# Tencent/PocketFlow

Hardware: AMD Instinct MI355X
Metric: images/sec ResNet-50 INT8 quant-aware fine-tune (whole job; per GPU = value / n_gpus) (higher is better)
Workload: dtype bf16

## Files before the change

### include/pocketflow_hip.h

```cpp
#ifndef POCKETFLOW_HIP_H_
#define POCKETFLOW_HIP_H_

#include <stdint.h>

#ifdef __cplusplus
extern "C" {
#endif

enum { PF_F32 = 0, PF_BF16 = 1 };
enum { PF_ACT_NONE = 0, PF_ACT_RELU = 1, PF_ACT_RELU6 = 2 };
enum { PF_BUCKET_TENSOR = 0, PF_BUCKET_CHANNEL = 1, PF_BUCKET_SPLIT = 2 };

typedef struct PfSeg {
  int64_t offset;
  int64_t len;
  int32_t RS;
  int32_t layout;
  int32_t I, O;
  int32_t mode;
  int32_t bits;
  int32_t bucket_size;
  int32_t n_bucket;
  int64_t slot_offset;
  int64_t cb_offset;
// ... 130 lines not shown

int pf_conv2d_stats_groups_geom(int imgs, int H, int Wd, int C, int N, int th, int tw, int stride, int pad_h, int pad_w,
                                int Ho, int Wo);
int pf_conv2d_fwd(const void* X, const void* W, void* Y, const void* zero, const void* R, float* partial,
                  const void* bn_x, const float* bn_scale_shift, const float* bn_mean_invstd, int bn_act,
                  int imgs, int H, int Wd, int C, int N, int th, int tw, int stride, int pad_h, int pad_w,
                  int Ho, int Wo, void* stream);
int pf_conv2d_fwd_affine(const void* X, const void* W, void* Y, const void* zero, const float* out_scale_shift, int out_act,
                         int imgs, int H, int Wd, int C, int N, int th, int tw, int stride, int pad_h, int pad_w, int Ho, int Wo,
                         void* stream);

int pf_conv2d_wrw_splits(int M, int N, int C, int taps);
int pf_conv2d_wrw(const void* dY, const void* X, void* dW, int dw_dtype, float* workspace, int imgs, int H, int Wd, int C,
                  int N, int th, int tw, int stride, int pad_h, int pad_w, int Ho, int Wo, void* stream);

typedef struct PfTransposeTile {
  int64_t src_off, dst_off;
  int32_t O, I, src_ld, dst_ld;
  int32_t o0, i0;
  int32_t reserved0, reserved1;
} PfTransposeTile;
int pf_seg_transpose(const void* src_flat, void* dst_flat, int dtype, const void* tiles, int n_tiles, void* stream);

int pf_maxpool_fwd(const void* x, void* y, void* idx, int dtype, int B, int H, int W, int C, int k, int stride,
                   int pad_h, int pad_w, int Ho, int Wo, void* stream);
int pf_maxpool_bwd(const void* dy, const void* idx, void* dx, int dtype, int B, int H, int W, int C, int k, int stride,
                   int pad_h, int pad_w, int Ho, int Wo, void* stream);

int pf_conv_stem_supported(int H, int Wd, int C, int N, int k, int stride, int pad);
int pf_conv_stem_fwd(const void* X, const void* W, void* Y, int imgs, int H, int Wd, void* stream);
// ... 101 lines not shown
```

### pocketflow_amd/csrc/pf_conv.hip

```cpp
#include "pf_conv_common.h"

template <int BN_T, bool PRO, bool BWD, bool MAP>
__global__ __launch_bounds__(PF_THREADS, 2) void k_conv1x1_fwd(const ConvArgs a) {
  constexpr int WM = (BN_T == 128) ? 64 : 32;
  constexpr int JM = WM / 16;
  constexpr int CS_LD = BN_T + 8;
  constexpr int VPR = BN_T / 8;
  constexpr int RPP = PF_THREADS / VPR;
  constexpr int NBV = BN_T * 8 / PF_THREADS;
  constexpr int A_EL = CV_BM * CV_LDK, B_EL = BN_T * CV_LDK;
  constexpr int C_EL = CV_BM * CS_LD;
  constexpr int RED_FL = 4 * RPP * BN_T;
  constexpr int SM_BYTES_AB = (A_EL + B_EL) * 2;
  constexpr int SM_BYTES = SM_BYTES_AB > RED_FL * 4 ? (SM_BYTES_AB > C_EL * 2 ? SM_BYTES_AB : C_EL * 2)
                                                    : RED_FL * 4;
  constexpr int SS_BYTES = PRO ? 2 * CV_MAXK * 4 : 0;
  __shared__ __attribute__((aligned(16))) unsigned char smem[SM_BYTES + SS_BYTES];
  float* ssl = reinterpret_cast<float*>(smem + SM_BYTES);
  __shared__ float bpl[BWD ? 4 * BN_T : 4];
  bf16_t* As = reinterpret_cast<bf16_t*>(smem);
  bf16_t* Bs = As + A_EL;
  bf16_t* Cs = reinterpret_cast<bf16_t*>(smem);
  float* red = reinterpret_cast<float*>(smem);

// ... 545 lines not shown
  if (e < n)
    for (int s = s0 + sg; s < s1; s += 4) acc += partial[(int64_t)s * n + e];
  l[sg][e_l] = acc;
  __syncthreads();
  if (sg == 0 && e < n) store_one<TO>(out + (int64_t)blockIdx.y * out_stride + e, (l[0][e_l] + l[1][e_l]) + (l[2][e_l] + l[3][e_l]));
}

WrwPlan pf_wrw_plan(int M, int N, int C, int taps, bool entry_1x1, int64_t x_rows, int window_imgs);
int pf_wrw2_launch(const void* dY, const void* X, float* slabs, const float* scale_shift, int act, const uint32_t* slot,
                   int bits, int M, int N, int C, int th, int tw, int H, int Wd, int Ho, int Wo, int stride, int pad_h,
                   int pad_w, int S, int64_t x_rows, hipStream_t st);
int pf_wrw_tr_launch(const void* dY, const void* X, float* slabs, const float* scale_shift, int act,
                     const uint32_t* slot, int bits, int M, int N, int C, int th, int tw, int H, int Wd, int Ho, int Wo,
                     int stride, int pad_h, int pad_w, int S, hipStream_t st);

int pf_wrw_reduce(float* workspace, int S, int64_t n, void* dW, int dw_dtype, hipStream_t st) {
  const int gx = (int)((n + 63) / 64);
  int ry = 1;
  while (ry < 32 && gx * ry < 1024 && ry * 8 <= S) ry *= 2;
  float* stage = workspace + (int64_t)S * n;
  if (ry > 1) {
    k_wrw_reduce<float><<<dim3(gx, ry), PF_THREADS, 0, st>>>(workspace, S, n, stage, n);
    if (dw_dtype == PF_F32) k_wrw_reduce<float><<<dim3(gx, 1), PF_THREADS, 0, st>>>(stage, ry, n, (float*)dW, 0);
    else if (dw_dtype == PF_BF16) k_wrw_reduce<bf16_t><<<dim3(gx, 1), PF_THREADS, 0, st>>>(stage, ry, n, (bf16_t*)dW, 0);
    else return (int)hipErrorInvalidValue;
  } else {
    if (dw_dtype == PF_F32) k_wrw_reduce<float><<<dim3(gx, 1), PF_THREADS, 0, st>>>(workspace, S, n, (float*)dW, 0);
    else if (dw_dtype == PF_BF16) k_wrw_reduce<bf16_t><<<dim3(gx, 1), PF_THREADS, 0, st>>>(workspace, S, n, (bf16_t*)dW, 0);
    else return (int)hipErrorInvalidValue;
  }
  PF_LAUNCH_CHECK();
  return 0;
}

int pf_wrw_scatter_splits(int M, int N, int K) {
  const int tiles = ((N + WR_TN - 1) / WR_TN) * ((K + WR_TK - 1) / WR_TK);
  int S = (768 + tiles - 1) / tiles;
  const int maxS = (M + 4 * WR_BM - 1) / (4 * WR_BM);
  if (S > maxS) S = maxS;
  if (S < 1) S = 1;
  int rows = (M + S - 1) / S;
  rows = ((rows + WR_BM - 1) / WR_BM) * WR_BM;
  return (M + rows - 1) / rows;
}

extern "C" int pf_conv1x1_wrw_splits(int M, int N, int K) { return pf_wrw_plan(M, N, K, 1, true, 0, 0).S; }

extern "C" int pf_conv1x1_wrw(const void* dY, const void* X, void* dW, int dw_dtype, float* workspace,
                              const float* scale_shift, int act, const uint32_t* slot, int bits, int M, int N,
                              int K, int Ho, int Wo, int H, int Wd, int stride, void* stream) {
  if (M <= 0 || N <= 0 || K <= 0 || (K % 8) || (N % 8) || ((int64_t)N * K) % 4) return (int)hipErrorInvalidValue;
  if (!pf_aligned16(dY) || !pf_aligned16(X) || !pf_aligned16(workspace) || !pf_aligned16(dW))
    return (int)hipErrorInvalidValue;
  if (slot != nullptr && (bits < 1 || bits > 32 || scale_shift == nullptr)) return (int)hipErrorInvalidValue;
  if (stride < 1) stride = 1;
  hipStream_t st = (hipStream_t)stream;
  if (stride > 1 && (Ho <= 0 || Wo <= 0 || H <= 0 || Wd <= 0)) return (int)hipErrorInvalidValue;
  const int64_t x_rows = (stride > 1) ? (int64_t)(M / (Ho * Wo)) * H * Wd : (int64_t)M;
  const WrwPlan p = pf_wrw_plan(M, N, K, 1, true, x_rows, 0);
  int r = 0;
  if (p.kernel == WRW_SHARED) {
    r = pf_wrw2_launch(dY, X, workspace, scale_shift, act, slot, bits, M, N, K, 1, 1, H, Wd, Ho, Wo, stride, 0, 0, p.S, x_rows, st);
  } else if (p.kernel == WRW_WAVE) {
    r = pf_wrw_tr_launch(dY, X, workspace, scale_shift, act, slot, bits, M, N, K, 1, 1, H, Wd, Ho, Wo, stride, 0, 0, p.S, st);
  } else {
    ConvArgs a = conv_args(X, dY, nullptr, M, N, K);
    conv_args_prologue(a, scale_shift, act, slot, bits);
    conv_args_rowmap(a, Ho, Wo, H, Wd, stride, 0);
    a.partial = workspace;
    a.tiles_n = (N + WR_TN - 1) / WR_TN;
    const int tiles_k = (K + WR_TK - 1) / WR_TK;
    int rows = (M + p.S - 1) / p.S;
    rows = ((rows + WR_BM - 1) / WR_BM) * WR_BM;
    a.rows_per_split = rows;
    dim3 grid(a.tiles_n * tiles_k, p.S);
    if (scale_shift != nullptr) k_conv1x1_wrw<true><<<grid, PF_THREADS, 0, st>>>(a);
    else k_conv1x1_wrw<false><<<grid, PF_THREADS, 0, st>>>(a);
    PF_LAUNCH_CHECK();
  }
  if (r != 0) return r;
  return pf_wrw_reduce(workspace, p.S, (int64_t)N * K, dW, dw_dtype, st);
}
```

### pocketflow_amd/csrc/pf_stem.hip

```cpp
#include "pf_conv_common.h"

#define LDS_PTR(p) ((__attribute__((address_space(3))) void*)(p))
typedef short st_v4s __attribute__((ext_vector_type(4)));
typedef short st_v8s __attribute__((ext_vector_type(8)));
#if defined(__HIP_DEVICE_COMPILE__)
typedef __amdgpu_buffer_rsrc_t st_rsrc_t;
#define ST_MAKE_RSRC(p, bytes) __builtin_amdgcn_make_buffer_rsrc((void*)(p), (short)0, (int)(bytes), 0x00020000)
#define ST_BUFFER_LOAD_LDS16(rs, lds, voff) __builtin_amdgcn_raw_ptr_buffer_load_lds(rs, LDS_PTR(lds), 16, voff, 0, 0, 0)
#else
typedef int st_rsrc_t;
#define ST_MAKE_RSRC(p, bytes) 0
#define ST_BUFFER_LOAD_LDS16(rs, lds, voff) ((void)(rs), (void)(lds), (void)(voff))
#endif

#define ST_THREADS 256
#define ST_OROWS 8
#define ST_IROWS (2 * ST_OROWS + 5)
#define ST_N 64
#define ST_R 7
#define ST_WL_BYTES (ST_N * ST_R * 32 * 2)

struct StemArgs {
  const bf16_t* X;
  const bf16_t* W;
// ... 240 lines not shown
}

int pf_wrw_reduce(float* workspace, int S, int64_t n, void* dW, int dw_dtype, hipStream_t st);

static int stem_wrw_grid(int imgs, int H) {
  const int items = imgs * ((H / 2 + SW_OROWS - 1) / SW_OROWS);
  return items < 768 ? items : 768;
}

extern "C" int pf_conv_stem_wrw_slabs(int imgs, int H, int Wd) {
  if (!pf_conv_stem_supported(H, Wd, 3, ST_N, 7, 2, 3) || imgs <= 0 || Wd > 256) return 0;
  if ((int64_t)imgs * (H / 2) * (Wd / 2) * ST_N * 2 >= (int64_t)1 << 31) return 0;
  return stem_wrw_grid(imgs, H);
}

extern "C" int pf_conv_stem_wrw(const void* dY, const void* X, void* dW, int dw_dtype, float* workspace, int imgs, int H,
                                int Wd, void* stream) {
  const int S = pf_conv_stem_wrw_slabs(imgs, H, Wd);
  if (S <= 0 || workspace == nullptr) return (int)hipErrorInvalidValue;
  if (!pf_aligned16(dY) || (reinterpret_cast<uintptr_t>(X) & 3u)) return (int)hipErrorInvalidValue;
  StemWrwArgs a;
  a.dY = (const bf16_t*)dY; a.X = (const bf16_t*)X; a.slabs = workspace;
  a.imgs = imgs; a.H = H; a.Wd = Wd; a.Ho = H / 2; a.Wo = Wd / 2;
  a.strips = (a.Ho + SW_OROWS - 1) / SW_OROWS;
  a.n_items = imgs * a.strips;
  a.rsb = (Wd + 8) * 8;
  a.dy_bytes = (int)((int64_t)imgs * a.Ho * a.Wo * ST_N * 2);
  const size_t lds = (size_t)SW_IROWS * a.rsb + (size_t)SW_OROWS * a.Wo * ST_N * 2;
  if (int e = pf_require_lds(reinterpret_cast<const void*>(&k_stem7x7_wrw), lds)) return e;
  k_stem7x7_wrw<<<S, ST_THREADS, lds, (hipStream_t)stream>>>(a);
  PF_LAUNCH_CHECK();
  return pf_wrw_reduce(workspace, S, (int64_t)ST_N * 147, dW, dw_dtype, (hipStream_t)stream);
}
```

### pocketflow_amd/csrc/pf_wrw.hip

```cpp
#include "pf_conv_common.h"
#include <stdlib.h>

#define LDS_PTR(p) ((__attribute__((address_space(3))) void*)(p))
typedef short v4s __attribute__((ext_vector_type(4)));
typedef short v8s __attribute__((ext_vector_type(8)));

__device__ __attribute__((aligned(16))) const uint32_t pf_wrw_zero_page[64] = {0};

struct WrwArgs {
  const bf16_t* dY;
  const bf16_t* X;
  float* slabs;
  const float* ss;
  const uint32_t* slot;
  float kq, act_lo, act_hi;
  int M, N, C;
  int th, tw, H, Wd, Ho, Wo, stride, pad_h, pad_w;
  int tiles_n, tiles, rows_per_split;
};

template <int N> __device__ __forceinline__ void wrw_wait_vm() { asm volatile("s_waitcnt vmcnt(%0)" ::"n"(N) : "memory"); }

template <int BN, bool PRO, bool MAP>
__global__ __launch_bounds__(256) void k_wrw_tr(const WrwArgs a) {
// ... 612 lines not shown
  const int s1 = (!entry_1x1 || pf_tuning().wrw_tr != 0) ? wrw_tr_splits(M, N, C, taps) : 0;
  if (s1 > 0) return WrwPlan{WRW_WAVE, s1};
  if (entry_1x1) return WrwPlan{WRW_SCATTER, pf_wrw_scatter_splits(M, N, C)};
  return WrwPlan{WRW_NONE, 0};
}

extern "C" int pf_conv2d_wrw_splits(int M, int N, int C, int taps) {
  const int s = pf_wrw_plan(M, N, C, taps, false, 0, 0).S;
  if (pf_tuning().conv3x3_c64 != 0 && taps == 9 && N == 64 && C == 64 && M % (56 * 56) == 0) {
    const int s3 = pf_wrw_plan(M, N, C, taps, false, 0, M / (56 * 56)).S;
    return s3 > s ? s3 : s;
  }
  return s;
}

extern "C" int pf_conv2d_wrw(const void* dY, const void* X, void* dW, int dw_dtype, float* workspace, int imgs, int H,
                             int Wd, int C, int N, int th, int tw, int stride, int pad_h, int pad_w, int Ho, int Wo,
                             void* stream) {
  if (imgs <= 0 || H <= 0 || Wd <= 0 || Ho <= 0 || Wo <= 0 || th < 1 || tw < 1 || stride < 1) return (int)hipErrorInvalidValue;
  if (!pf_aligned16(dY) || !pf_aligned16(X) || !pf_aligned16(dW) || !pf_aligned16(workspace)) return (int)hipErrorInvalidValue;
  const int M = imgs * Ho * Wo;
  hipStream_t st = (hipStream_t)stream;
  const bool window = pf_wrw3x3_c64_geom(H, Wd, C, N, th, tw, stride, pad_h, pad_w, Ho, Wo);
  const WrwPlan p = pf_wrw_plan(M, N, C, th * tw, false, (int64_t)imgs * H * Wd, window ? imgs : 0);
  int r = (int)hipErrorInvalidValue;
  if (p.kernel == WRW_WINDOW) r = pf_wrw3x3_c64_launch(dY, X, workspace, imgs, st);
  if (p.kernel == WRW_SHARED)
    r = pf_wrw2_launch(dY, X, workspace, nullptr, PF_ACT_NONE, nullptr, 8, M, N, C, th, tw, H, Wd, Ho, Wo, stride, pad_h, pad_w, p.S,
                       (int64_t)imgs * H * Wd, st);
  if (p.kernel == WRW_WAVE)
    r = pf_wrw_tr_launch(dY, X, workspace, nullptr, PF_ACT_NONE, nullptr, 8, M, N, C, th, tw, H, Wd, Ho, Wo, stride, pad_h, pad_w, p.S, st);
  if (r != 0) return r;
  return pf_wrw_reduce(workspace, p.S, (int64_t)N * th * tw * C, dW, dw_dtype, st);
}
```

### pocketflow_amd/graph.py

```python
from __future__ import annotations

import contextlib
import math
import os
import weakref
import threading
from dataclasses import dataclass, field
from typing import Callable, Dict, List, Optional, Sequence, Tuple

import numpy as np
import torch
import torch.nn.functional as F

from pocketflow_amd import hip
from pocketflow_amd.hip import check_gather
from pocketflow_amd.plan import WeightDesc
from pocketflow_amd.profiling import region

ALIGN = 64
FUSE_BN_BWD_STATS = os.environ.get('PF_FUSE_BN_BWD_STATS', '1') != '0'
HEAD_FUSE = os.environ.get('PF_HEAD_FUSE', '1') != '0'
HEAD_FUSE_ANY_DEVICE = False
BN_JOIN_ANY_DEVICE = False

# ... 62 lines not shown
      return WeightDesc(self.name, self.offset, s[0] * s[1], s[2], 1, 1)
    raise ValueError('not a matmul kernel: %s' % self.name)


class VarStore:

  def __init__(self, scope: str):
    self.scope = scope
    self.vars: List[Variable] = []
    self.by_name: Dict[str, Variable] = {}
    self.finalized = False
    self.device = None
    self.compute_dtype = torch.float32
    self.weight_decay = 0.0
    self.grad_hook = None

  def add(self, name: str, ref_shape, kind: str, trainable: bool = True, l2: bool = True,
          init=None) -> Variable:
    full = self.scope + '/' + name if self.scope else name
    if full in self.by_name:
      return self.by_name[full]
    if self.finalized:
      raise RuntimeError('variable %s created after the store was finalized' % full)
    v = Variable(full, tuple(int(d) for d in ref_shape), kind, trainable, l2 and trainable, init)
    v.numel = int(np.prod(v.ref_shape))
    v.group = 'W' if kind in ('conv', 'dense', 'depthwise') else ('O' if trainable else 'S')
    v.store = self
    self.vars.append(v)
    self.by_name[full] = v
    return v
# ... 307 lines not shown



WRW_SIDE = os.environ.get('PF_WRW_SIDE', '1') != '0'


class WrwSide(object):

  def __init__(self, device):
    self.device = device
    self.stream = torch.cuda.Stream(device=device)
    self.keep: List = []
    self._scratch: Optional[torch.Tensor] = None
    self.armed = False
    self.forks = 0

  def scratch(self, n_floats: int) -> torch.Tensor:
    if self._scratch is None or self._scratch.numel() < n_floats:
      with torch.cuda.stream(self.stream):
        self._scratch = torch.empty(max(n_floats, 1 << 20), dtype=torch.float32, device=self.device)
    return self._scratch

  def join(self) -> None:
    if self.forks:
      torch.cuda.current_stream(self.device).wait_stream(self.stream)
    self.keep.clear()
    self.forks = 0


class _WrwQueue(object):

  def __init__(self, graph, direct, tensors):
    side = getattr(getattr(graph, 'store', None), 'wrw_side', None)
    self.side = side if (side is not None and side.armed and direct and not torch.cuda.is_current_stream_capturing()) else None
    self.graph, self.tensors, self.ctx = graph, tensors, None

  def __enter__(self):
    if self.side is None:
      return self.graph.scratch
    side = self.side
    side.stream.wait_stream(torch.cuda.current_stream(side.device))
    side.keep.append(self.tensors)
    side.forks += 1
    self.ctx = torch.cuda.stream(side.stream)
    self.ctx.__enter__()
    return side.scratch

  def __exit__(self, *exc):
    if self.ctx is not None:
      self.ctx.__exit__(*exc)
    return False


def _wrw_queue(graph, direct, *tensors):
  return _WrwQueue(graph, direct, tensors)


@contextlib.contextmanager
def wrw_side_armed(store: 'VarStore'):
  if not (WRW_SIDE and store is not None and getattr(store, 'device', None) is not None and torch.device(store.device).type == 'cuda'):
    yield
    return
  side = getattr(store, 'wrw_side', None)
  if side is None:
    side = store.wrw_side = WrwSide(store.device)
  side.armed = True
  try:
    yield
  finally:
    side.armed = False
    side.join()



def _nhwc(x: torch.Tensor) -> torch.Tensor:
  if x.dim() == 4:
    return x.contiguous(memory_format=torch.channels_last)
  return x.contiguous()


def _bn_fast_ok(C: int) -> bool:
  if C % 8:
    return False
  G = C // 8
  if G < 8:
    return 8 % G == 0
# ... 399 lines not shown
  gview = _grad_view(params[0], C) if params is not None else None
  bview = _grad_view(params[1], C) if params is not None else None
  direct = gview is not None and bview is not None
  dgamma = gview if direct else torch.empty(C, dtype=torch.float32, device=x.device)
  dbeta = bview if direct else torch.empty(C, dtype=torch.float32, device=x.device)
  hip.bn_bwd_finalize(partial, nblk, C, dgamma, dbeta)
  dx = torch.empty_like(x)
  zero = graph.zero_row(C)[:C] if frozen else None
  name, traffic, launch, hw, tail = apply_pass
  with region(name, traffic):
    launch(dq, x, dx, rows, C, *hw, scale_shift, mean_invstd, zero if frozen else dgamma, zero if frozen else dbeta, act,
           *tail)
  return (dx, None, None) if direct else (dx, dgamma, dbeta)


def _filter_grad(graph, w, w_var, keep, name, nbytes, launch):
  gw = getattr(w, 'grad', None)
  direct = gw is not None and gw.shape == w.shape and gw.dtype == w.dtype and gw.permute(0, 2, 3, 1).is_contiguous()
  target = (gw.permute(0, 2, 3, 1) if direct
            else torch.empty((w.shape[0], w.shape[2], w.shape[3], w.shape[1]), dtype=w.dtype, device=w.device))
  with _wrw_queue(graph, direct, *keep) as scratch, region(name, nbytes):
    launch(target, scratch)
    if direct:
      graph.store.notify_grad(w_var)
  return None if direct else target.permute(0, 3, 1, 2)


def _bwd_data_weight(graph, w_var, w):
  if USE_SEG_TRANSPOSE and w_var is not None and w_var.store is graph.store and w_var.tensor is w:
    return graph.store.transposed(w_var)
  return w.detach().permute(0, 2, 3, 1).flip(1, 2).permute(3, 1, 2, 0).contiguous()


def _krsc(w, dtype):
  wk = w.detach().permute(0, 2, 3, 1)
  if not wk.is_contiguous() or wk.dtype != dtype:
    wk = wk.contiguous().to(dtype)
  return wk

# ... 61 lines not shown
  @staticmethod
  def backward(ctx, dy):
    x, w2d = ctx.saved_tensors
    lazy, stride, graph, has_res, w_shape = ctx.meta
    dy = _nhwc(dy)
    N, K = w2d.shape
    M, geom, _ = _conv1x1_geom(x.shape, stride)
    ss = lazy.scale_shift if lazy is not None else None
    quant = lazy is not None and lazy.bits is not None
    act = lazy.act if lazy is not None else None
    dx = dw = None
    if ctx.needs_input_grad[1]:
      S = hip.conv1x1_wrw_splits(M, N, K)

      def wrw(dwk, scratch):
        hip.conv1x1_wrw(dy, x, dwk.view(N, K), scratch((S + 32) * N * K), M, N, K, scale_shift=ss, act=act,
                        slot=lazy.slot if quant else None, bits=lazy.bits if quant else 8, geom=geom)
      dw = _filter_grad(graph, ctx.w_leaf, ctx.w_var, (dy, x, w2d, ss, lazy), 'conv1x1_wrw', float((M * K + M * N) * 2), wrw)
    if ctx.needs_input_grad[0]:
      wt = _bwd_data_weight(graph, ctx.w_var, ctx.w_leaf).view(K, N)
      fuse_stats = (FUSE_BN_BWD_STATS and lazy is not None and lazy.n_consumers == 1 and geom is None
                    and lazy.mean_invstd is not None and lazy.act in ('Relu', 'Relu6'))
      join = (JOIN_TWO_CONSUMERS and lazy is not None and lazy.join_ok and lazy.n_consumers == 2
              and lazy.n_grad_consumers == 2)
      second = join and lazy.pending is not None
      res = lazy.pending if (second and geom is None) else None
      join_entry = getattr(hip, 'conv1x1_bwd_data_join', None) if PROJ_JOIN else None
      compact = (join and not second and geom is not None and join_entry is not None and lazy.dense_out is not None
                 and hip.conv1x1_join_plan(x.shape[0] * x.shape[2] * x.shape[3], lazy.dense_out, K) != 0)
      rgeom = lazy.pending_geom if res is not None else None
      join_stats = (res is not None and join_entry is not None and PROJ_JOIN_STATS and FUSE_BN_BWD_STATS
                    and lazy.mean_invstd is not None and lazy.act in ('Relu', 'Relu6')
                    and hip.conv1x1_join_plan(M, N, K, True) != 0)
# ... 89 lines not shown

  @staticmethod
  def backward(ctx, dy):
    x, w = ctx.saved_tensors
    stride, pad, graph, bn_box = ctx.meta
    dy = _nhwc(dy)
    dx = dw = None
    N, C, R, S = w.shape
    B, _, H, W = x.shape
    Ho, Wo = dy.shape[2], dy.shape[3]
    if ctx.needs_input_grad[1]:
      splits = hip.conv2d_wrw_splits(B * Ho * Wo, N, C, R * S) if (OWN_CONV2D_WRW and C >= OWN_CONV2D_WRW_MIN_C) else 0
      nbytes = float((x.numel() + dy.numel()) * 2)
      if splits > 0:
        def wrw(dwk, scratch):
          hip.conv2d_wrw(dy, x, dwk, scratch((splits + 32) * N * R * S * C), B, H, W, C, N, R, S, stride, pad[0], pad[1], Ho, Wo)
        dw = _filter_grad(graph, w, ctx.w_var, (dy, x), 'conv2d_wrw', nbytes, wrw)
      elif OWN_CONV2D_WRW and OWN_CONV_GENERIC and x.is_cuda and dy.dtype == x.dtype and w.dtype == x.dtype:
        gs = hip.convg_wrw_splits(B, C, N, R, S, Ho, Wo)
        dwk = torch.empty((N, R, S, C), dtype=w.dtype, device=x.device)
        with region('conv2d_wrw', nbytes):
          hip.convg_wrw(dy, x, dwk, graph.scratch(gs * N * R * S * C), B, H, W, C, N, R, S, stride, pad[0], pad[1], Ho, Wo)
        dw = dwk.permute(0, 3, 1, 2)
      else:
        with region('conv2d_wrw', nbytes):
          dw = torch.ops.aten.convolution_backward(dy, x, w.detach(), None, [stride, stride], list(pad), [1, 1], False,
                                                   [0, 0], 1, [False, True, False])[1]
    if ctx.needs_input_grad[0]:
      mfma = N % 64 == 0 and C % 8 == 0 and igemm_limits_ok(dy.numel(), w.numel(), R * S)
      by_classes = (OWN_CONV2D_BWD_STRIDED and stride > 1 and H % stride == 0 and W % stride == 0 and R >= stride and S >= stride
                    and dy.dtype == torch.bfloat16)
      if mfma and (stride == 1 or by_classes):
# ... 158 lines not shown
    ctx.meta = (graph, w_var)
    return _run_stem(x, w)

  @staticmethod
  def backward(ctx, dy):
    x, w = ctx.saved_tensors
    graph, w_var = ctx.meta
    dy = _nhwc(dy)
    dx = dw = None
    if ctx.needs_input_grad[1]:
      B, _, H, Wd = x.shape
      S = hip.conv_stem_wrw_slabs(B, H, Wd) if OWN_CONV2D_WRW else 0
      nbytes = float((x.numel() + dy.numel()) * 2)
      if S > 0:
        def wrw(dwk, scratch):
          hip.conv_stem_wrw(dy, x, dwk, scratch((S + 32) * 64 * 147), B, H, Wd)
        dw = _filter_grad(graph, w, w_var, (dy, x), 'conv_stem_wrw', nbytes, wrw)
      else:
        with region('conv_stem_wrw', nbytes):
          dw = torch.ops.aten.convolution_backward(dy, x, w.detach(), None, [2, 2], [3, 3], [1, 1], False, [0, 0], 1,
                                                   [False, True, False])[1]
    if ctx.needs_input_grad[0]:
      dx = torch.ops.aten.convolution_backward(dy, x, w.detach(), None, [2, 2], [3, 3], [1, 1], False, [0, 0], 1,
                                               [True, False, False])[0]
    return dx, dw, None, None


def _run_stem3(x, w, pads, out_hw):
  B, _, H, Wd = x.shape
  N = w.shape[0]
  Ho, Wo = out_hw
  y = torch.empty((B, N, Ho, Wo), dtype=x.dtype, device=x.device, memory_format=torch.channels_last)
# ... 754 lines not shown
```

### pocketflow_amd/hip.py

```python
from __future__ import annotations

import ctypes
import os
from ctypes import c_float, c_int, c_int64, c_void_p

import numpy as np
import torch

_LIB_PATH = os.environ.get('PF_HIP_LIB') or os.path.join(os.path.dirname(os.path.abspath(__file__)), 'csrc', 'libpocketflow_hip.so')

PF_F32, PF_BF16 = 0, 1
PF_ACT_NONE, PF_ACT_RELU, PF_ACT_RELU6 = 0, 1, 2
PF_BUCKET_TENSOR, PF_BUCKET_CHANNEL, PF_BUCKET_SPLIT = 0, 1, 2
PF_CHUNK = 4096

SEG_DTYPE = np.dtype([('offset', '<i8'), ('len', '<i8'), ('RS', '<i4'), ('layout', '<i4'),
                      ('I', '<i4'), ('O', '<i4'), ('mode', '<i4'), ('bits', '<i4'),
                      ('bucket_size', '<i4'), ('n_bucket', '<i4'), ('slot_offset', '<i8'),
                      ('cb_offset', '<i8')])
BLOCK_DTYPE = np.dtype([('seg', '<i4'), ('chunk', '<i4'), ('row0', '<i4'), ('nrows', '<i4')])
assert SEG_DTYPE.itemsize == 64 and BLOCK_DTYPE.itemsize == 16

ACT_CODES = {None: PF_ACT_NONE, 'none': PF_ACT_NONE, 'Relu': PF_ACT_RELU, 'relu': PF_ACT_RELU,
             'Relu6': PF_ACT_RELU6, 'relu6': PF_ACT_RELU6}
# ... 12 lines not shown
    'pf_depthwise_wrw', 'pf_conv2d_stats_groups_geom', 'pf_tuning_reload',
    'pf_adam_flat_dev', 'pf_momentum_flat_dev', 'pf_set_floats',
    'pf_convg_fwd', 'pf_convg_bwd_data', 'pf_convg_small_splits', 'pf_convg_wrw_splits', 'pf_convg_wrw', 'pf_conv2d_bwd_data_strided',
    'pf_prox_groups', 'pf_prox_norms', 'pf_prox_apply', 'pf_im2col', 'pf_col2im',
    'pf_conv_stem3_supported', 'pf_conv_stem3_fwd', 'pf_conv_stem3_wrw_slabs', 'pf_conv_stem3_wrw',
    'pf_conv1x1_fwd_affine', 'pf_conv2d_fwd_affine', 'pf_conv2d_bwd_data_strided_stats_groups',
    'pf_conv2d_bwd_data_strided_bnstats',
    'pf_cpr_gather', 'pf_cpr_gram_ws', 'pf_cpr_gram', 'pf_cpr_ista', 'pf_cpr_lstsq_splits', 'pf_cpr_lstsq_step', 'pf_cpr_lstsq_resid',
    'pf_conv_gather_fwd',
    'pf_conv1x1_join_plan', 'pf_conv1x1_bwd_data_join',
    'pf_bn_act_quant_pool', 'pf_bn_bwd_stats_pooled', 'pf_bn_bwd_apply_pooled', 'pf_ce_distill_head', 'pf_ce_combine',
    'pf_bn_act_quant_codes', 'pf_conv_i8_supported', 'pf_conv_i8_fwd',
    'pf_dw_i8_supported', 'pf_dw_i8_fwd',
    'pf_bn_act_quant_static', 'pf_conv_i8_fwd_q', 'pf_dw_i8_fwd_q',
    'pf_bn_add_act_groups', 'pf_bn_add_act_fwd', 'pf_bn_add_act_bwd_gate', 'pf_bn_add_act_bwd_gate_add',
]


class HipLibraryMissing(RuntimeError):
  pass


def lib_path() -> str:
  return _LIB_PATH


def _load() -> ctypes.CDLL:
  if not os.path.exists(_LIB_PATH):
    raise HipLibraryMissing(
        'pocketflow_amd: %s not found -- build it with `python -c "import __graft_entry__ as g; '
# ... 412 lines not shown
  Ho, Wo, H, Wd, stride = geom if geom is not None else (0, 0, 0, 0, 1)
  if out_scale_shift is not None:
    if R is not None or partial is not None or slot is not None or ymap:
      raise ValueError('the folded output pass takes no residual, statistics, quantiser or row map')
    _check(_lib.pf_conv1x1_fwd_affine(_ptr(X), _ptr(W), _ptr(Y), _ptr(scale_shift), c_int(ACT_CODES[act]), _ptr(out_scale_shift),
                                      c_int(ACT_CODES[out_act]), c_int(M), c_int(N), c_int(K), c_int(Ho), c_int(Wo), c_int(H),
                                      c_int(Wd), c_int(stride), _stream()), 'pf_conv1x1_fwd_affine')
    return
  _check(_lib.pf_conv1x1_fwd(_ptr(X), _ptr(W), _ptr(Y), _ptr(R), _ptr(scale_shift), c_int(ACT_CODES[act]),
                             _ptr(slot), c_int(int(bits)), _ptr(partial), c_int(M), c_int(N), c_int(K), c_int(Ho),
                             c_int(Wo), c_int(H), c_int(Wd), c_int(stride), c_int(1 if ymap else 0), _stream()),
         'pf_conv1x1_fwd')


def conv1x1_wrw(dY, X, dW, workspace, M: int, N: int, K: int, scale_shift=None, act=None, slot=None,
                bits: int = 8, geom=None) -> None:
  _dev(X)
  Ho, Wo, H, Wd, stride = geom if geom is not None else (0, 0, 0, 0, 1)
  _check(_lib.pf_conv1x1_wrw(_ptr(dY), _ptr(X), _ptr(dW), c_int(dtype_code(dW)), _ptr(workspace), _ptr(scale_shift),
                             c_int(ACT_CODES[act]), _ptr(slot), c_int(int(bits)), c_int(M), c_int(N), c_int(K),
                             c_int(Ho), c_int(Wo), c_int(H), c_int(Wd), c_int(stride), _stream()), 'pf_conv1x1_wrw')


def conv1x1_bwd_data_bnstats(dY, Wt, dQ, bn_x, bn_scale_shift, bn_mean_invstd, bn_act, partial, M: int, N: int,
                             K: int) -> None:
  _dev(dY)
  _check(_lib.pf_conv1x1_bwd_data_bnstats(_ptr(dY), _ptr(Wt), _ptr(dQ), _ptr(bn_x), _ptr(bn_scale_shift),
                                          _ptr(bn_mean_invstd), c_int(ACT_CODES[bn_act]), _ptr(partial), c_int(M),
                                          c_int(N), c_int(K), _stream()), 'pf_conv1x1_bwd_data_bnstats')


def conv1x1_join_plan(M: int, N: int, K: int, with_stats: bool = False) -> int:
  return int(_lib.pf_conv1x1_join_plan(c_int(M), c_int(N), c_int(K), c_int(1 if with_stats else 0)))
# ... 38 lines not shown
                                     c_int(ACT_CODES[out_act]), c_int(imgs), c_int(H), c_int(Wd), c_int(C), c_int(N), c_int(th),
                                     c_int(tw), c_int(stride), c_int(pad_h), c_int(pad_w), c_int(Ho), c_int(Wo), _stream()),
           'pf_conv2d_fwd_affine')
    return
  _check(_lib.pf_conv2d_fwd(_ptr(X), _ptr(W), _ptr(Y), _ptr(zero_page(X.device)), _ptr(R), _ptr(partial), _ptr(bn_x),
                            _ptr(bn_scale_shift), _ptr(bn_mean_invstd), c_int(ACT_CODES[bn_act]), c_int(imgs), c_int(H),
                            c_int(Wd), c_int(C), c_int(N), c_int(th), c_int(tw), c_int(stride), c_int(pad_h),
                            c_int(pad_w), c_int(Ho), c_int(Wo), _stream()), 'pf_conv2d_fwd')


def conv2d_wrw_splits(M: int, N: int, C: int, taps: int) -> int:
  return int(_lib.pf_conv2d_wrw_splits(c_int(M), c_int(N), c_int(C), c_int(taps)))


def conv2d_wrw(dY, X, dW, workspace, imgs: int, H: int, Wd: int, C: int, N: int, th: int, tw: int, stride: int,
               pad_h: int, pad_w: int, Ho: int, Wo: int) -> None:
  _dev(X)
  _check(_lib.pf_conv2d_wrw(_ptr(dY), _ptr(X), _ptr(dW), c_int(dtype_code(dW)), _ptr(workspace), c_int(imgs), c_int(H),
                            c_int(Wd), c_int(C), c_int(N), c_int(th), c_int(tw), c_int(stride), c_int(pad_h),
                            c_int(pad_w), c_int(Ho), c_int(Wo), _stream()), 'pf_conv2d_wrw')


def depthwise_supported(C: int, k: int, stride: int) -> bool:
  return bool(_lib.pf_depthwise_supported(c_int(C), c_int(k), c_int(stride)))


def depthwise_groups(B: int, Ho: int, Wo: int, C: int) -> int:
  return int(_lib.pf_depthwise_groups(c_int(B), c_int(Ho), c_int(Wo), c_int(C)))


def depthwise_fwd(X, W, Y, B: int, H: int, Wd: int, C: int, k: int, stride: int, pad_h: int, pad_w: int, Ho: int, Wo: int,
                  partial=None) -> None:
  _dev(X)
  _check(_lib.pf_depthwise_fwd(_ptr(X), _ptr(W), _ptr(Y), c_int(dtype_code(X)), _ptr(partial), c_int(B), c_int(H), c_int(Wd),
                               c_int(C), c_int(k), c_int(stride), c_int(pad_h), c_int(pad_w), c_int(Ho), c_int(Wo),
# ... 258 lines not shown


def conv_stem_supported(H: int, Wd: int, C: int, N: int, k: int, stride: int, pad: int) -> bool:
  return bool(_lib.pf_conv_stem_supported(c_int(H), c_int(Wd), c_int(C), c_int(N), c_int(k), c_int(stride), c_int(pad)))


def conv_stem_fwd(X, W, Y, imgs: int, H: int, Wd: int) -> None:
  _dev(X)
  _check(_lib.pf_conv_stem_fwd(_ptr(X), _ptr(W), _ptr(Y), c_int(imgs), c_int(H), c_int(Wd), _stream()), 'pf_conv_stem_fwd')


def conv_stem_wrw_slabs(imgs: int, H: int, Wd: int) -> int:
  return int(_lib.pf_conv_stem_wrw_slabs(c_int(imgs), c_int(H), c_int(Wd)))


def conv_stem_wrw(dY, X, dW, workspace, imgs: int, H: int, Wd: int) -> None:
  _dev(dY)
  _check(_lib.pf_conv_stem_wrw(_ptr(dY), _ptr(X), _ptr(dW), c_int(dtype_code(dW)), _ptr(workspace), c_int(imgs), c_int(H),
                               c_int(Wd), _stream()), 'pf_conv_stem_wrw')


def conv_stem3_supported(H: int, Wd: int, C: int, N: int, k: int, stride: int, pad_h: int, pad_w: int, Ho: int, Wo: int) -> bool:
  return bool(_lib.pf_conv_stem3_supported(c_int(H), c_int(Wd), c_int(C), c_int(N), c_int(k), c_int(stride), c_int(pad_h), c_int(pad_w),
                                           c_int(Ho), c_int(Wo)))


def conv_stem3_fwd(X, W, Y, imgs: int, H: int, Wd: int, N: int, pad_h: int, pad_w: int, Ho: int, Wo: int) -> None:
  _dev(X)
  _check(_lib.pf_conv_stem3_fwd(_ptr(X), _ptr(W), _ptr(Y), c_int(imgs), c_int(H), c_int(Wd), c_int(N), c_int(pad_h), c_int(pad_w),
                                c_int(Ho), c_int(Wo), _stream()), 'pf_conv_stem3_fwd')


# ... 39 lines not shown
```

Before: 11710.

## Defer weight-gradient slab reductions into a batched multi-segment reduce kernel

Weight-gradient kernels (1x1, generic conv2d, stem) now only write per-split partial slabs into a pooled arena, and the final split reductions are queued and executed together in one batched kernel that walks a segment table. This replaces one or two small reduce launches per conv layer with a few large launches, cutting launch overhead and tail underutilisation. It costs extra arena memory (up to a configurable MB limit) and delays gradient availability until flush, which disables the path when grad hooks are present and may reduce overlap with the side stream.

```diff
diff --git a/include/pocketflow_hip.h b/include/pocketflow_hip.h
--- a/include/pocketflow_hip.h
+++ b/include/pocketflow_hip.h
@@ -168,6 +168,22 @@
 int pf_conv2d_wrw(const void* dY, const void* X, void* dW, int dw_dtype, float* workspace, int imgs, int H, int Wd, int C,
                   int N, int th, int tw, int stride, int pad_h, int pad_w, int Ho, int Wo, void* stream);
 
+typedef struct PfWrwSeg {
+  const float* slabs;
+  void* out;
+  int64_t n;
+  int32_t S;
+  int32_t dtype;
+} PfWrwSeg;
+int pf_conv1x1_wrw_write(const void* dY, const void* X, float* workspace, const float* scale_shift, int act,
+                         const uint32_t* slot, int bits, int M, int N, int K, int Ho, int Wo, int H, int Wd, int stride,
+                         int* S_out, void* stream);
+int pf_conv2d_wrw_write(const void* dY, const void* X, float* workspace, int imgs, int H, int Wd, int C, int N, int th, int tw,
+                        int stride, int pad_h, int pad_w, int Ho, int Wo, int* S_out, void* stream);
+int pf_conv_stem_wrw_write(const void* dY, const void* X, float* workspace, int imgs, int H, int Wd, void* stream);
+int pf_wrw_reduce_slabs(float* workspace, int S, int64_t n, void* dW, int dw_dtype, void* stream);
+int pf_wrw_reduce_batch(const PfWrwSeg* segs, int count, void* stream);
+
 typedef struct PfTransposeTile {
   int64_t src_off, dst_off;
   int32_t O, I, src_ld, dst_ld;
diff --git a/pocketflow_amd/csrc/pf_conv.hip b/pocketflow_amd/csrc/pf_conv.hip
--- a/pocketflow_amd/csrc/pf_conv.hip
+++ b/pocketflow_amd/csrc/pf_conv.hip
@@ -583,10 +583,112 @@
                      const uint32_t* slot, int bits, int M, int N, int C, int th, int tw, int H, int Wd, int Ho, int Wo,
                      int stride, int pad_h, int pad_w, int S, hipStream_t st);
 
-int pf_wrw_reduce(float* workspace, int S, int64_t n, void* dW, int dw_dtype, hipStream_t st) {
+#define WRB_SEGS 64
+struct WrwSegDev { const float* slabs; void* out; int64_t n; int S; int ry_dtype; };
+struct WrwBatchArgs { WrwSegDev seg[WRB_SEGS]; int wg_end[WRB_SEGS]; int count; };
+
+__device__ __forceinline__ float4 add4(float4 a, float4 b) { return make_float4(a.x + b.x, a.y + b.y, a.z + b.z, a.w + b.w); }
+
+__device__ __forceinline__ float4 wrb_range(const float* __restrict__ p, int64_t n, int s0, int s1) {
+  float4 l0 = make_float4(0.f, 0.f, 0.f, 0.f), l1 = l0, l2 = l0, l3 = l0;
+  int s = s0;
+#pragma unroll 2
+  for (; s + 4 <= s1; s += 4) {
+    const float4 v0 = *reinterpret_cast<const float4*>(p + (int64_t)s * n);
+    const float4 v1 = *reinterpret_cast<const float4*>(p + (int64_t)(s + 1) * n);
+    const float4 v2 = *reinterpret_cast<const float4*>(p + (int64_t)(s + 2) * n);
+    const float4 v3 = *reinterpret_cast<const float4*>(p + (int64_t)(s + 3) * n);
+    l0 = add4(l0, v0); l1 = add4(l1, v1); l2 = add4(l2, v2); l3 = add4(l3, v3);
+  }
+  if (s < s1) l0 = add4(l0, *reinterpret_cast<const float4*>(p + (int64_t)s * n));
+  if (s + 1 < s1) l1 = add4(l1, *reinterpret_cast<const float4*>(p + (int64_t)(s + 1) * n));
+  if (s + 2 < s1) l2 = add4(l2, *reinterpret_cast<const float4*>(p + (int64_t)(s + 2) * n));
+  return add4(add4(l0, l1), add4(l2, l3));
+}
+
+__global__ __launch_bounds__(PF_THREADS) void k_wrw_reduce_batch(const WrwBatchArgs a) {
+  __shared__ float4 l[4][64];
+  const int b = blockIdx.x;
+  int lo = 0, hi = a.count - 1;
+  while (lo < hi) {
+    const int mid = (lo + hi) >> 1;
+    if (b < a.wg_end[mid]) hi = mid; else lo = mid + 1;
+  }
+  const WrwSegDev sg = a.seg[lo];
+  const int wg = b - (lo > 0 ? a.wg_end[lo - 1] : 0);
+  const int lane = threadIdx.x & 63, w = threadIdx.x >> 6;
+  const int64_t e = ((int64_t)wg * 64 + lane) * 4;
+  const int ry = sg.ry_dtype & 0xFF;
+  float4 acc = make_float4(0.f, 0.f, 0.f, 0.f);
+  if (e < sg.n) {
+    const float* __restrict__ p = sg.slabs + e;
+    if (ry == 1) {
+      int s = w;
+      for (; s + 12 < sg.S; s += 16) {
+        const float4 v0 = *reinterpret_cast<const float4*>(p + (int64_t)s * sg.n);
+        const float4 v1 = *reinterpret_cast<const float4*>(p + (int64_t)(s + 4) * sg.n);
+        const float4 v2 = *reinterpret_cast<const float4*>(p + (int64_t)(s + 8) * sg.n);
+        const float4 v3 = *reinterpret_cast<const float4*>(p + (int64_t)(s + 12) * sg.n);
+        acc = add4(add4(add4(add4(acc, v0), v1), v2), v3);
+      }
+      for (; s < sg.S; s += 4) acc = add4(acc, *reinterpret_cast<const float4*>(p + (int64_t)s * sg.n));
+    } else {
+      const int per = (sg.S + ry - 1) / ry;
+      for (int y = w; y < ry; y += 4) {
+        const int s0 = y * per, s1 = (s0 + per < sg.S) ? (s0 + per) : sg.S;
+        acc = add4(acc, wrb_range(p, sg.n, s0, s1));
+      }
+    }
+  }
+  l[w][lane] = acc;
+  __syncthreads();
+  if (w == 0 && e < sg.n) {
+    const float4 r = add4(add4(l[0][lane], l[1][lane]), add4(l[2][lane], l[3][lane]));
+    if ((sg.ry_dtype >> 8) == PF_F32) {
+      *reinterpret_cast<float4*>((float*)sg.out + e) = r;
+    } else {
+      uint2 o;
+      o.x = (uint32_t)f32_to_bf16(r.x) | ((uint32_t)f32_to_bf16(r.y) << 16);
+      o.y = (uint32_t)f32_to_bf16(r.z) | ((uint32_t)f32_to_bf16(r.w) << 16);
+      *reinterpret_cast<uint2*>((bf16_t*)sg.out + e) = o;
+    }
+  }
+}
+
+static int wrw_reduce_ranges(int S, int64_t n) {
   const int gx = (int)((n + 63) / 64);
   int ry = 1;
   while (ry < 32 && gx * ry < 1024 && ry * 8 <= S) ry *= 2;
+  return ry;
+}
+
+extern "C" int pf_wrw_reduce_batch(const PfWrwSeg* segs, int count, void* stream) {
+  if (count < 0 || (count > 0 && segs == nullptr)) return (int)hipErrorInvalidValue;
+  for (int i = 0; i < count; ++i) {
+    const PfWrwSeg& s = segs[i];
+    if (s.S < 1 || s.n <= 0 || (s.n % 4) || (s.n + 255) / 256 > 0x3FFFFF || !pf_aligned16(s.slabs) || !pf_aligned16(s.out) ||
+        (s.dtype != PF_F32 && s.dtype != PF_BF16))
+      return (int)hipErrorInvalidValue;
+  }
+  for (int i0 = 0; i0 < count; i0 += WRB_SEGS) {
+    WrwBatchArgs a;
+    a.count = (count - i0 < WRB_SEGS) ? (count - i0) : WRB_SEGS;
+    int wgs = 0;
+    for (int i = 0; i < WRB_SEGS; ++i) {
+      const PfWrwSeg& s = segs[i0 + (i < a.count ? i : 0)];
+      a.seg[i] = WrwSegDev{s.slabs, s.out, s.n, s.S, wrw_reduce_ranges(s.S, s.n) | (s.dtype << 8)};
+      if (i < a.count) wgs += (int)((s.n + 255) / 256);
+      a.wg_end[i] = wgs;
+    }
+    k_wrw_reduce_batch<<<wgs, PF_THREADS, 0, (hipStream_t)stream>>>(a);
+    PF_LAUNCH_CHECK();
+  }
+  return 0;
+}
+
+int pf_wrw_reduce(float* workspace, int S, int64_t n, void* dW, int dw_dtype, hipStream_t st) {
+  const int gx = (int)((n + 63) / 64);
+  const int ry = wrw_reduce_ranges(S, n);
   float* stage = workspace + (int64_t)S * n;
   if (ry > 1) {
     k_wrw_reduce<float><<<dim3(gx, ry), PF_THREADS, 0, st>>>(workspace, S, n, stage, n);
@@ -602,6 +704,11 @@
   return 0;
 }
 
+extern "C" int pf_wrw_reduce_slabs(float* workspace, int S, int64_t n, void* dW, int dw_dtype, void* stream) {
+  if (S < 1 || n <= 0 || (n % 4) || !pf_aligned16(workspace) || !pf_aligned16(dW)) return (int)hipErrorInvalidValue;
+  return pf_wrw_reduce(workspace, S, n, dW, dw_dtype, (hipStream_t)stream);
+}
+
 int pf_wrw_scatter_splits(int M, int N, int K) {
   const int tiles = ((N + WR_TN - 1) / WR_TN) * ((K + WR_TK - 1) / WR_TK);
   int S = (768 + tiles - 1) / tiles;
@@ -615,12 +722,11 @@
 
 extern "C" int pf_conv1x1_wrw_splits(int M, int N, int K) { return pf_wrw_plan(M, N, K, 1, true, 0, 0).S; }
 
-extern "C" int pf_conv1x1_wrw(const void* dY, const void* X, void* dW, int dw_dtype, float* workspace,
-                              const float* scale_shift, int act, const uint32_t* slot, int bits, int M, int N,
-                              int K, int Ho, int Wo, int H, int Wd, int stride, void* stream) {
+extern "C" int pf_conv1x1_wrw_write(const void* dY, const void* X, float* workspace, const float* scale_shift, int act,
+                                    const uint32_t* slot, int bits, int M, int N, int K, int Ho, int Wo, int H, int Wd,
+                                    int stride, int* S_out, void* stream) {
   if (M <= 0 || N <= 0 || K <= 0 || (K % 8) || (N % 8) || ((int64_t)N * K) % 4) return (int)hipErrorInvalidValue;
-  if (!pf_aligned16(dY) || !pf_aligned16(X) || !pf_aligned16(workspace) || !pf_aligned16(dW))
-    return (int)hipErrorInvalidValue;
+  if (!pf_aligned16(dY) || !pf_aligned16(X) || !pf_aligned16(workspace) || S_out == nullptr) return (int)hipErrorInvalidValue;
   if (slot != nullptr && (bits < 1 || bits > 32 || scale_shift == nullptr)) return (int)hipErrorInvalidValue;
   if (stride < 1) stride = 1;
   hipStream_t st = (hipStream_t)stream;
@@ -648,5 +754,15 @@
     PF_LAUNCH_CHECK();
   }
   if (r != 0) return r;
-  return pf_wrw_reduce(workspace, p.S, (int64_t)N * K, dW, dw_dtype, st);
-}
+  *S_out = p.S;
+  return 0;
+}
+
+extern "C" int pf_conv1x1_wrw(const void* dY, const void* X, void* dW, int dw_dtype, float* workspace,
+                              const float* scale_shift, int act, const uint32_t* slot, int bits, int M, int N,
+                              int K, int Ho, int Wo, int H, int Wd, int stride, void* stream) {
+  if (!pf_aligned16(dW)) return (int)hipErrorInvalidValue;
+  int S = 0;
+  if (int r = pf_conv1x1_wrw_write(dY, X, workspace, scale_shift, act, slot, bits, M, N, K, Ho, Wo, H, Wd, stride, &S, stream)) return r;
+  return pf_wrw_reduce(workspace, S, (int64_t)N * K, dW, dw_dtype, (hipStream_t)stream);
+}
diff --git a/pocketflow_amd/csrc/pf_stem.hip b/pocketflow_amd/csrc/pf_stem.hip
--- a/pocketflow_amd/csrc/pf_stem.hip
+++ b/pocketflow_amd/csrc/pf_stem.hip
@@ -278,8 +278,7 @@
   return stem_wrw_grid(imgs, H);
 }
 
-extern "C" int pf_conv_stem_wrw(const void* dY, const void* X, void* dW, int dw_dtype, float* workspace, int imgs, int H,
-                                int Wd, void* stream) {
+extern "C" int pf_conv_stem_wrw_write(const void* dY, const void* X, float* workspace, int imgs, int H, int Wd, void* stream) {
   const int S = pf_conv_stem_wrw_slabs(imgs, H, Wd);
   if (S <= 0 || workspace == nullptr) return (int)hipErrorInvalidValue;
   if (!pf_aligned16(dY) || (reinterpret_cast<uintptr_t>(X) & 3u)) return (int)hipErrorInvalidValue;
@@ -294,5 +293,11 @@
   if (int e = pf_require_lds(reinterpret_cast<const void*>(&k_stem7x7_wrw), lds)) return e;
   k_stem7x7_wrw<<<S, ST_THREADS, lds, (hipStream_t)stream>>>(a);
   PF_LAUNCH_CHECK();
-  return pf_wrw_reduce(workspace, S, (int64_t)ST_N * 147, dW, dw_dtype, (hipStream_t)stream);
-}
+  return 0;
+}
+
+extern "C" int pf_conv_stem_wrw(const void* dY, const void* X, void* dW, int dw_dtype, float* workspace, int imgs, int H,
+                                int Wd, void* stream) {
+  if (int r = pf_conv_stem_wrw_write(dY, X, workspace, imgs, H, Wd, stream)) return r;
+  return pf_wrw_reduce(workspace, pf_conv_stem_wrw_slabs(imgs, H, Wd), (int64_t)ST_N * 147, dW, dw_dtype, (hipStream_t)stream);
+}
diff --git a/pocketflow_amd/csrc/pf_wrw.hip b/pocketflow_amd/csrc/pf_wrw.hip
--- a/pocketflow_amd/csrc/pf_wrw.hip
+++ b/pocketflow_amd/csrc/pf_wrw.hip
@@ -650,11 +650,10 @@
   return s;
 }
 
-extern "C" int pf_conv2d_wrw(const void* dY, const void* X, void* dW, int dw_dtype, float* workspace, int imgs, int H,
-                             int Wd, int C, int N, int th, int tw, int stride, int pad_h, int pad_w, int Ho, int Wo,
-                             void* stream) {
+extern "C" int pf_conv2d_wrw_write(const void* dY, const void* X, float* workspace, int imgs, int H, int Wd, int C, int N, int th,
+                                   int tw, int stride, int pad_h, int pad_w, int Ho, int Wo, int* S_out, void* stream) {
   if (imgs <= 0 || H <= 0 || Wd <= 0 || Ho <= 0 || Wo <= 0 || th < 1 || tw < 1 || stride < 1) return (int)hipErrorInvalidValue;
-  if (!pf_aligned16(dY) || !pf_aligned16(X) || !pf_aligned16(dW) || !pf_aligned16(workspace)) return (int)hipErrorInvalidValue;
+  if (!pf_aligned16(dY) || !pf_aligned16(X) || !pf_aligned16(workspace) || S_out == nullptr) return (int)hipErrorInvalidValue;
   const int M = imgs * Ho * Wo;
   hipStream_t st = (hipStream_t)stream;
   const bool window = pf_wrw3x3_c64_geom(H, Wd, C, N, th, tw, stride, pad_h, pad_w, Ho, Wo);
@@ -667,5 +666,15 @@
   if (p.kernel == WRW_WAVE)
     r = pf_wrw_tr_launch(dY, X, workspace, nullptr, PF_ACT_NONE, nullptr, 8, M, N, C, th, tw, H, Wd, Ho, Wo, stride, pad_h, pad_w, p.S, st);
   if (r != 0) return r;
-  return pf_wrw_reduce(workspace, p.S, (int64_t)N * th * tw * C, dW, dw_dtype, st);
-}
+  *S_out = p.S;
+  return 0;
+}
+
+extern "C" int pf_conv2d_wrw(const void* dY, const void* X, void* dW, int dw_dtype, float* workspace, int imgs, int H,
+                             int Wd, int C, int N, int th, int tw, int stride, int pad_h, int pad_w, int Ho, int Wo,
+                             void* stream) {
+  if (!pf_aligned16(dW)) return (int)hipErrorInvalidValue;
+  int S = 0;
+  if (int r = pf_conv2d_wrw_write(dY, X, workspace, imgs, H, Wd, C, N, th, tw, stride, pad_h, pad_w, Ho, Wo, &S, stream)) return r;
+  return pf_wrw_reduce(workspace, S, (int64_t)N * th * tw * C, dW, dw_dtype, (hipStream_t)stream);
+}
diff --git a/pocketflow_amd/graph.py b/pocketflow_amd/graph.py
--- a/pocketflow_amd/graph.py
+++ b/pocketflow_amd/graph.py
@@ -100,6 +100,7 @@
     self.compute_dtype = torch.float32
     self.weight_decay = 0.0
     self.grad_hook = None
+    self.wrw_deferred = 0
 
   def add(self, name: str, ref_shape, kind: str, trainable: bool = True, l2: bool = True,
           init=None) -> Variable:
@@ -437,6 +438,7 @@
     self._scratch: Optional[torch.Tensor] = None
     self.armed = False
     self.forks = 0
+    self.arena: Optional['WrwArena'] = None
 
   def scratch(self, n_floats: int) -> torch.Tensor:
     if self._scratch is None or self._scratch.numel() < n_floats:
@@ -445,16 +447,95 @@
     return self._scratch
 
   def join(self) -> None:
+    if self.arena is not None and self.arena.pending and self.arena.side is self:
+      with torch.cuda.stream(self.stream):
+        self.arena.flush()
     if self.forks:
       torch.cuda.current_stream(self.device).wait_stream(self.stream)
     self.keep.clear()
     self.forks = 0
 
 
+WRW_BATCH = os.environ.get('PF_WRW_BATCH', '1') != '0'
+WRW_BATCH_MB = float(os.environ.get('PF_WRW_BATCH_MB', '128'))
+
+
+class _ArenaFull(Exception):
+  pass
+
+
+class WrwArena(object):
+
+  CHUNK = 64 << 20
+
+  def __init__(self, store):
+    self.store = store
+    self.chunks: List[torch.Tensor] = []
+    self.cur = self.off = 0
+    self.pending: List[tuple] = []
+    self.pending_bytes = 0
+    self.limit = int(WRW_BATCH_MB * (1 << 20))
+    self.side: Optional[WrwSide] = None
+    self.armed = False
+    self.flushes = 0
+
+  def bytes(self) -> int:
+    return sum(c.numel() for c in self.chunks) * 4
+
+  def _fit(self, n: int) -> Optional[torch.Tensor]:
+    while self.cur < len(self.chunks):
+      c = self.chunks[self.cur]
+      if self.off + n <= c.numel():
+        t = c[self.off:self.off + n]
+        self.off += n
+        return t
+      self.cur, self.off = self.cur + 1, 0
+    return None
+
+  def take(self, n_floats: int) -> torch.Tensor:
+    n = (int(n_floats) + 63) & ~63
+    t = self._fit(n)
+    if t is None and torch.cuda.is_current_stream_capturing():
+      self.flush()
+      t = self._fit(n)
+      if t is None:
+        raise _ArenaFull()
+    if t is None:
+      self.chunks.append(torch.empty(max(n, self.CHUNK), dtype=torch.float32, device=self.store.device))
+      t = self._fit(n)
+    self._taken = t
+    return t
+
+  def defer(self, side, launch, target) -> bool:
+    self.side = side
+    try:
+      S = launch(None, self.take)
+    except _ArenaFull:
+      return False
+    n = target.numel()
+    self.pending.append((self._taken.data_ptr(), int(S), n, target.data_ptr(), hip.dtype_code(target)))
+    self.pending_bytes += int(S) * n * 4
+    self.store.wrw_deferred += 1
+    if self.limit and self.pending_bytes >= self.limit:
+      self.flush()
+    return True
+
+  def flush(self) -> None:
+    if self.pending:
+      hip.wrw_reduce_batch(sorted(self.pending, key=lambda s: -s[1]))
+      self.flushes += 1
+    self.pending = []
+    self.pending_bytes = 0
+    self.cur = self.off = 0
+
+
 class _WrwQueue(object):
 
   def __init__(self, graph, direct, tensors):
-    side = getattr(getattr(graph, 'store', None), 'wrw_side', None)
+    store = getattr(graph, 'store', None)
+    side = getattr(store, 'wrw_side', None)
+    arena = getattr(store, 'wrw_arena', None)
+    self.arena = arena if (arena is not None and arena.armed and direct and store.grad_hook is None) else None
     self.side = side if (side is not None and side.armed and direct and not torch.cuda.is_current_stream_capturing()) else None
     self.graph, self.tensors, self.ctx = graph, tensors, None
 
@@ -481,18 +562,30 @@
 
 @contextlib.contextmanager
 def wrw_side_armed(store: 'VarStore'):
-  if not (WRW_SIDE and store is not None and getattr(store, 'device', None) is not None and torch.device(store.device).type == 'cuda'):
+  if not ((WRW_SIDE or WRW_BATCH) and store is not None and getattr(store, 'device', None) is not None
+          and torch.device(store.device).type == 'cuda'):
     yield
     return
+  arena = getattr(store, 'wrw_arena', None)
+  if arena is None and WRW_BATCH:
+    arena = store.wrw_arena = WrwArena(store)
   side = getattr(store, 'wrw_side', None)
-  if side is None:
+  if side is None and WRW_SIDE:
     side = store.wrw_side = WrwSide(store.device)
-  side.armed = True
+  if side is not None:
+    side.armed, side.arena = True, arena
+  if arena is not None:
+    arena.armed = True
   try:
     yield
   finally:
-    side.armed = False
-    side.join()
+    if arena is not None:
+      arena.armed = False
+    if side is not None:
+      side.armed = False
+      side.join()
+    if arena is not None:
+      arena.flush()
 
 
 
@@ -922,15 +1015,17 @@
   return (dx, None, None) if direct else (dx, dgamma, dbeta)
 
 
-def _filter_grad(graph, w, w_var, keep, name, nbytes, launch):
+def _filter_grad(graph, w, w_var, keep, name, nbytes, launch, slabs=False):
   gw = getattr(w, 'grad', None)
   direct = gw is not None and gw.shape == w.shape and gw.dtype == w.dtype and gw.permute(0, 2, 3, 1).is_contiguous()
   target = (gw.permute(0, 2, 3, 1) if direct
             else torch.empty((w.shape[0], w.shape[2], w.shape[3], w.shape[1]), dtype=w.dtype, device=w.device))
-  with _wrw_queue(graph, direct, *keep) as scratch, region(name, nbytes):
-    launch(target, scratch)
-    if direct:
-      graph.store.notify_grad(w_var)
+  q = _wrw_queue(graph, direct, *keep)
+  with q as scratch, region(name, nbytes):
+    if not (slabs and q.arena is not None and q.arena.defer(q.side, launch, target)):
+      launch(target, scratch)
+      if direct:
+        graph.store.notify_grad(w_var)
   return None if direct else target.permute(0, 3, 1, 2)
 
 
@@ -1022,9 +1117,11 @@
       S = hip.conv1x1_wrw_splits(M, N, K)
 
       def wrw(dwk, scratch):
-        hip.conv1x1_wrw(dy, x, dwk.view(N, K), scratch((S + 32) * N * K), M, N, K, scale_shift=ss, act=act,
-                        slot=lazy.slot if quant else None, bits=lazy.bits if quant else 8, geom=geom)
-      dw = _filter_grad(graph, ctx.w_leaf, ctx.w_var, (dy, x, w2d, ss, lazy), 'conv1x1_wrw', float((M * K + M * N) * 2), wrw)
+        return hip.conv1x1_wrw(dy, x, dwk.view(N, K) if dwk is not None else None, scratch((S + (32 if dwk is not None else 0)) * N * K),
+                               M, N, K, scale_shift=ss, act=act, slot=lazy.slot if quant else None,
+                               bits=lazy.bits if quant else 8, geom=geom)
+      dw = _filter_grad(graph, ctx.w_leaf, ctx.w_var, (dy, x, w2d, ss, lazy), 'conv1x1_wrw', float((M * K + M * N) * 2), wrw,
+                        slabs=True)
     if ctx.needs_input_grad[0]:
       wt = _bwd_data_weight(graph, ctx.w_var, ctx.w_leaf).view(K, N)
       fuse_stats = (FUSE_BN_BWD_STATS and lazy is not None and lazy.n_consumers == 1 and geom is None
@@ -1144,8 +1241,9 @@
       nbytes = float((x.numel() + dy.numel()) * 2)
       if splits > 0:
         def wrw(dwk, scratch):
-          hip.conv2d_wrw(dy, x, dwk, scratch((splits + 32) * N * R * S * C), B, H, W, C, N, R, S, stride, pad[0], pad[1], Ho, Wo)
-        dw = _filter_grad(graph, w, ctx.w_var, (dy, x), 'conv2d_wrw', nbytes, wrw)
+          return hip.conv2d_wrw(dy, x, dwk, scratch((splits + (32 if dwk is not None else 0)) * N * R * S * C), B, H, W, C, N, R, S,
+                                stride, pad[0], pad[1], Ho, Wo)
+        dw = _filter_grad(graph, w, ctx.w_var, (dy, x), 'conv2d_wrw', nbytes, wrw, slabs=True)
       elif OWN_CONV2D_WRW and OWN_CONV_GENERIC and x.is_cuda and dy.dtype == x.dtype and w.dtype == x.dtype:
         gs = hip.convg_wrw_splits(B, C, N, R, S, Ho, Wo)
         dwk = torch.empty((N, R, S, C), dtype=w.dtype, device=x.device)
@@ -1334,8 +1432,8 @@
       nbytes = float((x.numel() + dy.numel()) * 2)
       if S > 0:
         def wrw(dwk, scratch):
-          hip.conv_stem_wrw(dy, x, dwk, scratch((S + 32) * 64 * 147), B, H, Wd)
-        dw = _filter_grad(graph, w, w_var, (dy, x), 'conv_stem_wrw', nbytes, wrw)
+          return hip.conv_stem_wrw(dy, x, dwk, scratch((S + (32 if dwk is not None else 0)) * 64 * 147), B, H, Wd)
+        dw = _filter_grad(graph, w, w_var, (dy, x), 'conv_stem_wrw', nbytes, wrw, slabs=True)
       else:
         with region('conv_stem_wrw', nbytes):
           dw = torch.ops.aten.convolution_backward(dy, x, w.detach(), None, [2, 2], [3, 3], [1, 1], False, [0, 0], 1,
diff --git a/pocketflow_amd/hip.py b/pocketflow_amd/hip.py
--- a/pocketflow_amd/hip.py
+++ b/pocketflow_amd/hip.py
@@ -50,6 +50,7 @@
     'pf_dw_i8_supported', 'pf_dw_i8_fwd',
     'pf_bn_act_quant_static', 'pf_conv_i8_fwd_q', 'pf_dw_i8_fwd_q',
     'pf_bn_add_act_groups', 'pf_bn_add_act_fwd', 'pf_bn_add_act_bwd_gate', 'pf_bn_add_act_bwd_gate_add',
+    'pf_conv1x1_wrw_write', 'pf_conv2d_wrw_write', 'pf_conv_stem_wrw_write', 'pf_wrw_reduce_slabs', 'pf_wrw_reduce_batch',
 ]
 
 
@@ -492,9 +493,15 @@
 
 
 def conv1x1_wrw(dY, X, dW, workspace, M: int, N: int, K: int, scale_shift=None, act=None, slot=None,
-                bits: int = 8, geom=None) -> None:
+                bits: int = 8, geom=None):
   _dev(X)
   Ho, Wo, H, Wd, stride = geom if geom is not None else (0, 0, 0, 0, 1)
+  if dW is None:
+    S = c_int(0)
+    _check(_lib.pf_conv1x1_wrw_write(_ptr(dY), _ptr(X), _ptr(workspace), _ptr(scale_shift), c_int(ACT_CODES[act]), _ptr(slot),
+                                     c_int(int(bits)), c_int(M), c_int(N), c_int(K), c_int(Ho), c_int(Wo), c_int(H), c_int(Wd),
+                                     c_int(stride), ctypes.byref(S), _stream()), 'pf_conv1x1_wrw_write')
+    return S.value
   _check(_lib.pf_conv1x1_wrw(_ptr(dY), _ptr(X), _ptr(dW), c_int(dtype_code(dW)), _ptr(workspace), _ptr(scale_shift),
                              c_int(ACT_CODES[act]), _ptr(slot), c_int(int(bits)), c_int(M), c_int(N), c_int(K),
                              c_int(Ho), c_int(Wo), c_int(H), c_int(Wd), c_int(stride), _stream()), 'pf_conv1x1_wrw')
@@ -563,11 +570,36 @@
 
 
 def conv2d_wrw(dY, X, dW, workspace, imgs: int, H: int, Wd: int, C: int, N: int, th: int, tw: int, stride: int,
-               pad_h: int, pad_w: int, Ho: int, Wo: int) -> None:
-  _dev(X)
+               pad_h: int, pad_w: int, Ho: int, Wo: int):
+  _dev(X)
+  if dW is None:
+    S = c_int(0)
+    _check(_lib.pf_conv2d_wrw_write(_ptr(dY), _ptr(X), _ptr(workspace), c_int(imgs), c_int(H), c_int(Wd), c_int(C), c_int(N),
+                                    c_int(th), c_int(tw), c_int(stride), c_int(pad_h), c_int(pad_w), c_int(Ho), c_int(Wo),
+                                    ctypes.byref(S), _stream()), 'pf_conv2d_wrw_write')
+    return S.value
   _check(_lib.pf_conv2d_wrw(_ptr(dY), _ptr(X), _ptr(dW), c_int(dtype_code(dW)), _ptr(workspace), c_int(imgs), c_int(H),
                             c_int(Wd), c_int(C), c_int(N), c_int(th), c_int(tw), c_int(stride), c_int(pad_h),
                             c_int(pad_w), c_int(Ho), c_int(Wo), _stream()), 'pf_conv2d_wrw')
+
+
+class WrwSeg(ctypes.Structure):
+  _fields_ = [('slabs', c_void_p), ('out', c_void_p), ('n', c_int64), ('S', ctypes.c_int32), ('dtype', ctypes.c_int32)]
+
+
+def wrw_reduce_slabs(workspace, S: int, n: int, dW) -> None:
+  _dev(workspace)
+  _check(_lib.pf_wrw_reduce_slabs(_ptr(workspace), c_int(S), c_int64(n), _ptr(dW), c_int(dtype_code(dW)), _stream()),
+         'pf_wrw_reduce_slabs')
+
+
+def wrw_reduce_batch(segs) -> None:
+  if not segs:
+    return
+  table = (WrwSeg * len(segs))()
+  for t, (slabs, S, n, out, code) in zip(table, segs):
+    t.slabs, t.out, t.n, t.S, t.dtype = slabs, out, n, S, code
+  _check(_lib.pf_wrw_reduce_batch(table, c_int(len(segs)), _stream()), 'pf_wrw_reduce_batch')
 
 
 def depthwise_supported(C: int, k: int, stride: int) -> bool:
@@ -856,8 +888,12 @@
   return int(_lib.pf_conv_stem_wrw_slabs(c_int(imgs), c_int(H), c_int(Wd)))
 
 
-def conv_stem_wrw(dY, X, dW, workspace, imgs: int, H: int, Wd: int) -> None:
+def conv_stem_wrw(dY, X, dW, workspace, imgs: int, H: int, Wd: int):
   _dev(dY)
+  if dW is None:
+    _check(_lib.pf_conv_stem_wrw_write(_ptr(dY), _ptr(X), _ptr(workspace), c_int(imgs), c_int(H), c_int(Wd), _stream()),
+           'pf_conv_stem_wrw_write')
+    return conv_stem_wrw_slabs(imgs, H, Wd)
   _check(_lib.pf_conv_stem_wrw(_ptr(dY), _ptr(X), _ptr(dW), c_int(dtype_code(dW)), _ptr(workspace), c_int(imgs), c_int(H),
                                c_int(Wd), _stream()), 'pf_conv_stem_wrw')
 
```

Result: no change. 11730 (median of 2 runs) (+0.1%).
